# javahedi/SpinDynamics.jl

Measured on AMD Instinct MI355X. Metric: H|psi> matvecs/s, XXZ L=32 Sz=0, higher is better.
Workload: dtype c128

## Files before the change

spindynamics.jl_amd/csrc/kernels_apply.hip:

```cpp
#include <hip/hip_runtime.h>

#include <algorithm>
#include <type_traits>

#include "device_common.hpp"


using namespace sd_dev;

namespace {

template <int NC, int R, int BLOCK, bool FMA, bool PK, bool GEN = false>
__global__ __launch_bounds__(BLOCK, (GEN ? 5 : NC == 2 ? 4 : 5)) void k_apply_tiled(sd_dev_model dm, double *__restrict__ out_,
                                                       const double *__restrict__ psi_, int epi, sd_epi_args ea,
                                                       double *__restrict__ partials, int max_len) {
  using V = typename VT<NC>::type;
  constexpr uint32_t ES = sizeof(V);
  constexpr int WR = R * 64;
  extern __shared__ __attribute__((aligned(16))) unsigned char smem[];
  V *tile = reinterpret_cast<V *>(smem);
  int *lbin = reinterpret_cast<int *>(smem + (size_t)(max_len + 1) * sizeof(V));
  double *red = reinterpret_cast<double *>(lbin + 16 * SD_BIN_STRIDE);
  V *tile2 = reinterpret_cast<V *>(red + 32);

  if (ea.batch > 1) {
    const int64_t boff = (int64_t)blockIdx.y * ea.bstride * NC;
    psi_ += boff; out_ += boff;
    if (ea.prev) ea.prev = (const double *)ea.prev + boff;
    if (ea.phi) ea.phi = (const double *)ea.phi + boff;
    if (ea.accv) ea.accv = (double *)ea.accv + boff;
    partials += 2 * (size_t)blockIdx.y * (size_t)dm.n_singles;
    ea.negate = (ea.negate >> blockIdx.y) & 1;
  }
  const V *__restrict__ psi = reinterpret_cast<const V *>(psi_);
  const V *__restrict__ halo = reinterpret_cast<const V *>(ea.halo);
  const int tid = threadIdx.x;
  const int lane = tid & 63;
  const int i0 = (tid >> 6) * WR + lane;
  const int tix = blockIdx.x + dm.tile_off;
  const sd_tile_rec rec = dm.single_rec[tix];
  const uint32_t P = rec.prefix;
  const int64_t base = rec.base;
  const int p = dm.p, LS = dm.LS;
  const int len = rec.len;
  const int nU = rec.nU;
  const int nn = dm.nn_hops;
  static_assert(!GEN || PK, "general-bond plan: packed tables only");
  const bool need_sig = GEN ? (dm.need_sig_gen != 0) : (!PK || dm.need_sig);

  V own[R];
  uint32_t sig[R];
  typedef unsigned int u4 __attribute__((ext_vector_type(4)));
  u4 pt[PK ? R : 1];
  uint32_t dg[R];
  const uint32_t off0 = (uint32_t)i0 * ES;
  {
    const __amdgpu_buffer_rsrc_t rs = make_rsrc(psi + base, (uint32_t)len * ES);
#pragma unroll
    for (int r = 0; r < R; ++r) buf_load(own[r], rs, off0 + (uint32_t)(r * 64) * ES);
    if (PK && !need_sig && !dm.diag_cache) {
      const __amdgpu_buffer_rsrc_t rg = make_rsrc(dm.suf_dg + rec.suf_off, (uint32_t)len);
#pragma unroll
      for (int r = 0; r < R; ++r) dg[r] = (uint32_t)(unsigned char)__builtin_amdgcn_raw_buffer_load_b8(rg, (uint32_t)i0 + (uint32_t)(r * 64), 0, 0);
    }
    if (need_sig) {
      const __amdgpu_buffer_rsrc_t rsig = make_rsrc(dm.suf_states + rec.suf_off, (uint32_t)len * 2u);
#pragma unroll
      for (int r = 0; r < R; ++r) sig[r] = buf_load_u16(rsig, (uint32_t)i0 * 2u + (uint32_t)(r * 64) * 2u);
    } else {
#pragma unroll
      for (int r = 0; r < R; ++r) sig[r] = 0;
    }
  }

  uint64_t fmask = 0;
  int64_t my_base = -1;
  const uint32_t bitp = p >= 1 ? ((P >> (p - 1)) & 1u) : 0u;
  if (nn > 0 && p >= 1) {
    const int b = lane + 1;
    if (b <= p) my_base = dm.far_base[(size_t)tix * (size_t)p + (size_t)lane];
    fmask = __ballot(my_base >= 0);
  }
  const int st_lo = bitp ? nU : 0, st_n = bitp ? len - nU : nU;
  auto get_bond = [&](int ln) {
    FarBond fb;
    fb.base = rl64(my_base, ln); fb.J = dm.hop_J[ln];
    const bool st = ln == p - 1;
    fb.lo = st ? st_lo : 0; fb.n = st ? st_n : len;
    return fb;
  };
  constexpr bool SKIP_DEAD = NC == 1 || BLOCK == 64;
  uint32_t live = 0;
  if (SKIP_DEAD) {
#pragma unroll
    for (int r = 0; r < R; ++r)
      if ((tid & ~63) / 64 * WR + r * 64 < len) live |= 1u << r;
    live = (uint32_t)__builtin_amdgcn_readfirstlane((int)live);
  }
  auto issue = [&](const FarBond &fb, V(&v)[R]) {
    const V *__restrict__ pb = (halo && fb.base >= dm.n_local) ? halo + (fb.base - dm.n_local) : psi + fb.base;
    const __amdgpu_buffer_rsrc_t rs = make_rsrc(pb, (uint32_t)fb.n * ES);
    const uint32_t rel = off0 - (uint32_t)fb.lo * ES;
#pragma unroll
    for (int r = 0; r < R; ++r)
      if (!SKIP_DEAD || ((live >> r) & 1u)) buf_load(v[r], rs, rel + (uint32_t)(r * 64) * ES);
  };

  V va[R], vb[R];
  if (SKIP_DEAD) {
#pragma unroll
    for (int r = 0; r < R; ++r) { va[r] = V{}; vb[r] = V{}; }
  }
  FarBond fa{}, fbb{};
  uint64_t mk = fmask;
  bool have_a = false;
  auto next_lane = [&](uint64_t &m_) { const int ln = __builtin_ctzll(m_); m_ &= m_ - 1; return ln; };
  if (mk) { fa = get_bond(next_lane(mk)); issue(fa, va); have_a = true; }

  V acc[R];
  if (dm.diag_cache) {
    double dd[R];
    const __amdgpu_buffer_rsrc_t rd = make_rsrc(dm.diag_cache + base, (uint32_t)len * (uint32_t)sizeof(double));
#pragma unroll
    for (int r = 0; r < R; ++r) buf_load(dd[r], rd, (uint32_t)i0 * (uint32_t)sizeof(double) + (uint32_t)(r * 64) * (uint32_t)sizeof(double));
#pragma unroll
    for (int r = 0; r < R; ++r) acc[r] = vscale(dd[r], own[r]);
  } else if (!need_sig) {
    const int antiP = p >= 2 ? __popc((P ^ (P >> 1)) & ((1u << (p - 1)) - 1u)) : 0;
#pragma unroll
    for (int r = 0; r < R; ++r) {
      int anti = antiP + (int)(dg[r] & 15u) + (p >= 1 ? (int)(bitp ^ (dg[r] >> 4)) : 0);
      if (dm.n_zz_nn == 0) anti = 0;
      acc[r] = vscale(dm.diag_q * (double)(dm.n_zz - 2 * anti), own[r]);
    }
  } else if (dm.diag_mode == 0) {
    const DiagHead dh = diag_head(dm, P, p);
#pragma unroll
    for (int r = 0; r < R; ++r) {
      const uint64_t s = (uint64_t)P | ((uint64_t)sig[r] << p);
      acc[r] = vscale(diag_tail(dm, dh, s, p), own[r]);
    }
  } else {
#pragma unroll
    for (int r = 0; r < R; ++r) {
      const uint64_t s = (uint64_t)P | ((uint64_t)sig[r] << p);
      acc[r] = vscale(diag_of(dm, s), own[r]);
    }
  }
#pragma unroll
  for (int r = 0; r < R; ++r)
    if (i0 + r * 64 < len) tile[1 + i0 + r * 64] = own[r];
  if (tid == 0) tile[0] = V{};
  if (!PK)
    for (int k = tid; k < 16 * SD_BIN_STRIDE; k += BLOCK) {
      int n = k / SD_BIN_STRIDE, kk = k - n * SD_BIN_STRIDE;
      lbin[k] = (int)binom_g(dm, n, kk);
    }

  __syncthreads();
  while (have_a) {
    bool have_b = false;
    if (mk) { fbb = get_bond(next_lane(mk)); issue(fbb, vb); have_b = true; }
#pragma unroll
    for (int r = 0; r < R; ++r) acc[r] = accum<FMA>(acc[r], fa.J, va[r]);
    have_a = false;
    if (!have_b) break;
    if (mk) { fa = get_bond(next_lane(mk)); issue(fa, va); have_a = true; }
#pragma unroll
    for (int r = 0; r < R; ++r) acc[r] = accum<FMA>(acc[r], fbb.J, vb[r]);
  }
  if (PK && nn > 0) {
    const __amdgpu_buffer_rsrc_t rp = make_rsrc(dm.suf_part + 4 * (size_t)rec.suf_off, (uint32_t)len * 16u);
#pragma unroll
    for (int r = 0; r < R; ++r) pt[PK ? r : 0] = __builtin_amdgcn_raw_buffer_load_b128(rp, (uint32_t)i0 * 16u + (uint32_t)(r * 64) * 16u, 0, 0);
  }
  const bool wrap = !GEN && PK && !(NC == 1 && R == 8) && nn > 0 && dm.wrap_hop == nn;
  bool wrap_on = false;
  if (wrap) {
    const uint32_t Q = P ^ (1u << dm.wrap_pb);
    const int t2q = dm.nup - __popc(Q);
    if (t2q >= 0 && t2q <= LS) {
      wrap_on = true;
      const int64_t qb = dm.addr[Q];
      const int lenq = (int)dm.binom[LS * (SD_MAX_L + 1) + t2q];
      const V *__restrict__ pbq = (halo && qb >= dm.n_local) ? halo + (qb - dm.n_local) : psi + qb;
      const __amdgpu_buffer_rsrc_t rq = make_rsrc(pbq, (uint32_t)lenq * ES);
      for (int c0 = 0; c0 < lenq; c0 += BLOCK * R) {
#pragma unroll
        for (int r = 0; r < R; ++r) buf_load(va[r], rq, off0 + (uint32_t)(c0 + r * 64) * ES);
#pragma unroll
        for (int r = 0; r < R; ++r)
          if (c0 + i0 + r * 64 < lenq) tile2[1 + c0 + i0 + r * 64] = va[r];
      }
      if (tid == 0) tile2[0] = V{};
    }
  }

  struct GBond { int64_t base; uint32_t smask; int pb; int kind; };
  auto gbond = [&](int h) {
    GBond g{0, 0u, 0, -1};
    const int bi = dm.hop_i[h] - 1, bj = dm.hop_j[h] - 1;
    const bool ip = bi < p, jp = bj < p;
    if (ip && jp) {
      if (((P >> bi) ^ (P >> bj)) & 1u) { g.kind = 0; g.base = dm.addr[P ^ (1u << bi) ^ (1u << bj)]; }
    } else if (!ip && !jp) {
      g.kind = 1; g.smask = (1u << (bi - p)) | (1u << (bj - p));
    } else {
      g.pb = ip ? bi : bj;
      g.smask = 1u << ((ip ? bj : bi) - p);
      const uint32_t Q = P ^ (1u << g.pb);
      const int t2q = dm.nup - __popc(Q);
      if (t2q >= 0 && t2q <= LS) { g.kind = 2; g.base = dm.addr[Q]; }
    }
    return g;
  };
  auto gflip = [&](const GBond &g, int r) -> bool {
    if (g.kind == 0) return true;
    if (g.kind == 1) return __popc(sig[r] & g.smask) == 1;
    if (g.kind == 2) return ((P >> g.pb) & 1u) != ((sig[r] & g.smask) ? 1u : 0u);
    return false;
  };
  auto gvalue = [&](const GBond &g, int r) -> V {
    if (g.kind == 1) return tile[1 + dm.suf_rank[sig[r] ^ g.smask]];
    const int64_t idx = g.base + (g.kind == 0 ? (int64_t)(i0 + r * 64) : (int64_t)dm.suf_rank[sig[r] ^ g.smask]);
    return (halo && idx >= dm.n_local) ? halo[idx - dm.n_local] : psi[idx];
  };
  const bool have_g = !GEN && nn < dm.n_hop;
  double gJ = 0.0;
  GBond g0{0, 0u, 0, -1};
  auto request_g0 = [&]() {
    g0 = gbond(nn);
    gJ = dm.hop_J[nn];
#pragma unroll
    for (int r = 0; r < R; ++r) va[r] = (i0 + r * 64 < len && gflip(g0, r)) ? gvalue(g0, r) : V{};
  };
  if (have_g && !PK) request_g0();
  if (nn > 0) {
    if constexpr (PK) {
      const unsigned char *tb = reinterpret_cast<const unsigned char *>(tile);
      constexpr uint32_t SH = NC == 2 ? 4 : 3;
#pragma unroll
      for (int a = 1; a <= 11; ++a) if (a <= LS - 1) {
        const double J = dm.hop_J[p + a - 1];
        const int w = (a - 1) / 3, sh = 10 * ((a - 1) % 3);
        V v[R];
#pragma unroll
        for (int r = 0; r < R; ++r) {
          const u4 q = pt[PK ? r : 0];
          const uint32_t word = w == 0 ? q.x : w == 1 ? q.y : w == 2 ? q.z : q.w;
          const uint32_t ad = ((word >> sh) & 0x3FFu) << SH;
          v[r] = *reinterpret_cast<const V *>(tb + ad);
        }
#pragma unroll
        for (int r = 0; r < R; ++r) acc[r] = accum<FMA>(acc[r], J, v[r]);
      }
    } else {
      uint32_t dw[R];
#pragma unroll
      for (int r = 0; r < R; ++r) dw[r] = sig[r] ^ (sig[r] >> 1);
      for (int a = 1; a <= LS - 1; ++a) {
        const double J = dm.hop_J[p + a - 1];
        const int *brow = lbin + (LS - a - 1) * SD_BIN_STRIDE;
        int d[R];
#pragma unroll
        for (int r = 0; r < R; ++r) d[r] = brow[__popc(sig[r] >> (a + 1))];
        V v[R];
#pragma unroll
        for (int r = 0; r < R; ++r) {
          const bool up = (sig[r] >> (a - 1)) & 1u;
          const bool fl = (dw[r] >> (a - 1)) & 1u;
          const int ip = (i0 + r * 64) + (up ? d[r] : -d[r]);
          v[r] = tile[fl ? ip + 1 : 0];
        }
#pragma unroll
        for (int r = 0; r < R; ++r) acc[r] = accum<FMA>(acc[r], J, v[r]);
      }
    }
  }
  if constexpr (GEN) {
    constexpr uint32_t SH = NC == 2 ? 4 : 3;
    const unsigned char *tb = reinterpret_cast<const unsigned char *>(tile);
    const unsigned char *tb2 = reinterpret_cast<const unsigned char *>(tile2);
    uint32_t ptw[R];
    int cur_word = -1;
    auto gissue = [&](int64_t gbase, V(&v)[R]) {
      const V *__restrict__ pbp = (halo && gbase >= dm.n_local) ? halo + (gbase - dm.n_local) : psi + gbase;
      const __amdgpu_buffer_rsrc_t rs = make_rsrc(pbp, (uint32_t)len * ES);
#pragma unroll
      for (int r = 0; r < R; ++r) buf_load(v[r], rs, off0 + (uint32_t)(r * 64) * ES);
    };
    for (int hb = 0; hb < dm.n_gen; hb += 64) {
      const int nb = dm.n_gen - hb < 64 ? dm.n_gen - hb : 64;
      int64_t base_k = -1;
      sd_gbond gl{-1, 0u, 0, 0, 0.0};
      if (lane < nb) {
        gl = dm.gen[hb + lane];
        if (gl.kind == 0 && __popc(P & gl.pmask) == 1) base_k = dm.addr[P ^ gl.pmask];
      }
      uint64_t todo = __ballot(base_k >= 0);
      int in_a = -1;
      if (todo) { in_a = next_lane(todo); gissue(rl64(base_k, in_a), va); }
#pragma nounroll
      for (int k = 0; k < nb; ++k) {
        sd_gbond gb;
        gb.kind = rl(gl.kind, k); gb.pmask = (uint32_t)rl((int)gl.pmask, k); gb.slot = rl(gl.slot, k); gb.pb = rl(gl.pb, k);
        gb.J = rld(gl.J, k);
        if (gb.kind == 0) {
          if (k == in_a) {
#pragma unroll
            for (int r = 0; r < R; ++r) acc[r] = accum<false>(acc[r], gb.J, va[r]);
            in_a = -1;
            if (todo) { in_a = next_lane(todo); gissue(rl64(base_k, in_a), va); }
          }
        } else if (gb.kind == 1) {
          const int wi = gb.slot / 3, sh = 10 * (gb.slot - 3 * wi);
          if (wi != cur_word) {
            cur_word = wi;
            const int chunk = wi >> 2;
            const __amdgpu_buffer_rsrc_t rp2 = make_rsrc(dm.gen_ss_part + 4 * ((size_t)chunk * (size_t)dm.n_suf_rows + (size_t)rec.suf_off), (uint32_t)len * 16u);
            const uint32_t wo = (uint32_t)(wi & 3) * 4u;
#pragma unroll
            for (int r = 0; r < R; ++r) ptw[r] = (uint32_t)__builtin_amdgcn_raw_buffer_load_b32(rp2, (uint32_t)i0 * 16u + (uint32_t)(r * 64) * 16u + wo, 0, 0);
          }
          V v[R];
#pragma unroll
          for (int r = 0; r < R; ++r) v[r] = *reinterpret_cast<const V *>(tb + ((((ptw[r] >> sh) & 0x3FFu)) << SH));
#pragma unroll
          for (int r = 0; r < R; ++r) acc[r] = accum<false>(acc[r], gb.J, v[r]);
        } else if (gb.kind == 2) {
          const uint32_t Q = P ^ gb.pmask;
          const int t2q = dm.nup - __popc(Q);
          const bool ok = t2q >= 0 && t2q <= LS;
          __syncthreads();
          if (ok) {
            const int64_t qb = dm.addr[Q];
            const int lenq = (int)dm.binom[LS * (SD_MAX_L + 1) + t2q];
            const V *__restrict__ pbq = (halo && qb >= dm.n_local) ? halo + (qb - dm.n_local) : psi + qb;
            const __amdgpu_buffer_rsrc_t rq = make_rsrc(pbq, (uint32_t)lenq * ES);
            for (int c0 = 0; c0 < lenq; c0 += BLOCK * R) {
              V tmp[R];
#pragma unroll
              for (int r = 0; r < R; ++r) buf_load(tmp[r], rq, off0 + (uint32_t)(c0 + r * 64) * ES);
#pragma unroll
              for (int r = 0; r < R; ++r)
                if (c0 + i0 + r * 64 < lenq) tile2[1 + c0 + i0 + r * 64] = tmp[r];
            }
            if (tid == 0) tile2[0] = V{};
          }
          __syncthreads();
          if (ok) {
            const __amdgpu_buffer_rsrc_t rm = make_rsrc(dm.mix_part + ((size_t)gb.slot * (size_t)dm.n_suf_rows + (size_t)rec.suf_off), (uint32_t)len * 2u);
            const uint32_t bpb = (P >> gb.pb) & 1u;
            uint32_t w16[R];
#pragma unroll
            for (int r = 0; r < R; ++r) w16[r] = buf_load_u16(rm, (uint32_t)i0 * 2u + (uint32_t)(r * 64) * 2u);
#pragma unroll
            for (int r = 0; r < R; ++r) {
              const bool has = (w16[r] >> 15) != bpb;
              const uint32_t ad = has ? ((w16[r] & 0x3FFu) << SH) : 0u;
              acc[r] = accum<false>(acc[r], gb.J, *reinterpret_cast<const V *>(tb2 + ad));
            }
          }
        }
      }
    }
  }
  if (wrap) {
    __syncthreads();
    if (wrap_on) {
      const double Jw = dm.hop_J[nn];
      const uint32_t bpb = (P >> dm.wrap_pb) & 1u;
      const unsigned char *tb2 = reinterpret_cast<const unsigned char *>(tile2);
      constexpr uint32_t SH = NC == 2 ? 4 : 3;
#pragma unroll
      for (int r = 0; r < R; ++r) {
        const uint32_t w3 = pt[PK ? r : 0].w;
        const bool has = ((w3 >> 30) & 1u) != bpb;
        const uint32_t ad = has ? (((w3 >> 20) & 0x3FFu) << SH) : 0u;
        acc[r] = accum<false>(acc[r], Jw, *reinterpret_cast<const V *>(tb2 + ad));
      }
    }
  }
  if (have_g) {
    if (!wrap) {
      if (PK) request_g0();
#pragma unroll
      for (int r = 0; r < R; ++r)
        if (gflip(g0, r)) acc[r] = accum<false>(acc[r], gJ, va[r]);
    }
    for (int h = nn + 1; h < dm.n_hop; ++h) {
      const GBond g = gbond(h);
      if (g.kind < 0) continue;
      const double J = dm.hop_J[h];
#pragma unroll
      for (int r = 0; r < R; ++r)
        if (i0 + r * 64 < len && gflip(g, r)) acc[r] = accum<false>(acc[r], J, gvalue(g, r));
    }
  }

  EpiSums sums{0.0, 0.0};
#pragma unroll
  for (int r = 0; r < R; ++r) {
    const int i = i0 + r * 64;
    if (i < len) epilogue<NC>(epi, ea, base + i, acc[r], tile[1 + i], out_, sums);
  }
  if (epi_has_sums(epi)) {
    double a = sums.s0, b = sums.s1;
    block_reduce2(a, b, red);
    if (tid == 0) { partials[2 * (size_t)tix] = a; partials[2 * (size_t)tix + 1] = b; }
  }
}

template <int NC, bool FMA>
__global__ __launch_bounds__(256, 4) void k_apply_fulltile(sd_dev_model dm, double *__restrict__ out_,
                                                        const double *__restrict__ psi_, int epi, sd_epi_args ea,
                                                        double *__restrict__ partials) {
  using V = typename VT<NC>::type;
  constexpr uint32_t ES = sizeof(V);
  constexpr int R = 4, BLOCK = 256;
  extern __shared__ __attribute__((aligned(16))) unsigned char smem[];
  const int LF = dm.full_ls, TL = 1 << LF;
  V *tile = reinterpret_cast<V *>(smem);
  double *red = reinterpret_cast<double *>(smem + (size_t)(TL + 1) * sizeof(V));
  const V *__restrict__ psi = reinterpret_cast<const V *>(psi_);
  const V *__restrict__ halo = reinterpret_cast<const V *>(ea.halo);
  const int tid = threadIdx.x, lane = tid & 63;
  uint32_t T = blockIdx.x;
  if (gridDim.x >= 512 && (gridDim.x & 255u) == 0) {
    const uint32_t x = T & 7u, j = T >> 3, g = j >> 5, i = j & 31u;
    T = (g << 8) + (x << 5) + i;
  }
  const int64_t base = (int64_t)T << LF;
  const uint32_t Tg = T + (uint32_t)(dm.row_lo >> LF);
  const int64_t gbase = (int64_t)Tg << LF;
  const int nn = dm.nn_hops;

  V own[R];
  uint32_t ioff[R];
  {
    const __amdgpu_buffer_rsrc_t rs = make_rsrc(psi + base, (uint32_t)TL * ES);
#pragma unroll
    for (int r = 0; r < R; ++r) { ioff[r] = (uint32_t)(tid + r * BLOCK) * ES; buf_load(own[r], rs, ioff[r]); }
  }
  uint64_t fmask = 0;
  int64_t my_base = 0;
  double my_J = 0.0;
  int my_lo = 0, my_n = TL;
  if (nn > 0) {
    const int a = LF + lane;
    bool fl = false;
    if (a <= dm.L - 1) {
      if (lane == 0) {
        const int t = (int)(T & 1u);
        my_lo = (1 - t) * (TL / 2); my_n = TL / 2;
        my_base = ((int64_t)(T ^ 1u) << LF) + (TL / 2 - my_lo);
        fl = true;
      } else {
        const int b = a - LF - 1;
        fl = ((Tg >> b) ^ (Tg >> (b + 1))) & 1u;
        const uint32_t Tp = Tg ^ (3u << b);
        const int tb = dm.L - LF - dm.fs_dbits;
        const uint32_t q = Tp >> tb;
        const int64_t at_peer = (int64_t)(Tp & ((1u << tb) - 1u)) << LF;
        my_base = at_peer;
        if (q != (Tg >> tb)) {
          int64_t ho = 0, plo = 0;
#pragma unroll
          for (int q2 = 0; q2 < SD_FS_MAX_RANKS; ++q2)
            if ((uint32_t)q2 == q) { ho = dm.fs_halo_off[q2]; plo = dm.fs_peer_lo[q2]; }
          my_base = dm.n_local + ho + at_peer - plo;
        }
      }
      my_J = dm.hop_J[a - 1];
    }
    fmask = __ballot(fl);
  }
  auto get_bond = [&](int ln) {
    FarBond fb;
    fb.base = rl64(my_base, ln); fb.J = rld(my_J, ln);
    fb.lo = rl(my_lo, ln); fb.n = rl(my_n, ln);
    return fb;
  };
  auto issue = [&](const FarBond &fb, V(&v)[R]) {
    const V *__restrict__ pb = (halo && fb.base >= dm.n_local) ? halo + (fb.base - dm.n_local) : psi + fb.base;
    const __amdgpu_buffer_rsrc_t rs = make_rsrc(pb, (uint32_t)fb.n * ES);
    const uint32_t lo_b = (uint32_t)fb.lo * ES;
#pragma unroll
    for (int r = 0; r < R; ++r) buf_load(v[r], rs, ioff[r] - lo_b);
  };
  V va[R], vb[R];
  FarBond fa{}, fbb{};
  uint64_t mk = fmask;
  bool have_a = false;
  auto next_lane = [&](uint64_t &m_) { const int ln = __builtin_ctzll(m_); m_ &= m_ - 1; return ln; };
  if (mk) { fa = get_bond(next_lane(mk)); issue(fa, va); have_a = true; }

  V acc[R];
#pragma unroll
  for (int r = 0; r < R; ++r) {
    acc[r] = vscale(diag_of(dm, (uint64_t)gbase + (uint64_t)(tid + r * BLOCK)), own[r]);
    tile[tid + r * BLOCK] = own[r];
  }
  if (tid == 0) tile[TL] = V{};
  __syncthreads();

  const int n_in = nn > 0 ? LF - 1 : 0;
  for (int a = 1; a <= n_in; ++a) {
    const double J = dm.hop_J[a - 1];
    V v[R];
#pragma unroll
    for (int r = 0; r < R; ++r) {
      const int i = tid + r * BLOCK;
      const bool fl = ((i >> (a - 1)) ^ (i >> a)) & 1;
      v[r] = tile[fl ? (i ^ (3 << (a - 1))) : TL];
    }
#pragma unroll
    for (int r = 0; r < R; ++r) acc[r] = accum<FMA>(acc[r], J, v[r]);
  }
  while (have_a) {
    bool have_b = false;
    if (mk) { fbb = get_bond(next_lane(mk)); issue(fbb, vb); have_b = true; }
#pragma unroll
    for (int r = 0; r < R; ++r) acc[r] = accum<FMA>(acc[r], fa.J, va[r]);
    have_a = false;
    if (!have_b) break;
    if (mk) { fa = get_bond(next_lane(mk)); issue(fa, va); have_a = true; }
#pragma unroll
    for (int r = 0; r < R; ++r) acc[r] = accum<FMA>(acc[r], fbb.J, vb[r]);
  }
  for (int h = nn; h < dm.n_hop; ++h) {
    const int bi = dm.hop_i[h] - 1, bj = dm.hop_j[h] - 1;
    const double J = dm.hop_J[h];
#pragma unroll
    for (int r = 0; r < R; ++r) {
      const uint64_t s = (uint64_t)gbase + (uint64_t)(tid + r * BLOCK);
      if (((s >> bi) ^ (s >> bj)) & 1) acc[r] = accum<false>(acc[r], J, psi[s ^ ((uint64_t)1 << bi) ^ ((uint64_t)1 << bj)]);
    }
  }
  EpiSums sums{0.0, 0.0};
#pragma unroll
  for (int r = 0; r < R; ++r) {
    const int i = tid + r * BLOCK;
    epilogue<NC>(epi, ea, base + i, acc[r], tile[i], out_, sums);
  }
  if (epi_has_sums(epi)) {
    double a = sums.s0, b = sums.s1;
    block_reduce2(a, b, red);
    if (tid == 0) { partials[2 * (size_t)blockIdx.x] = a; partials[2 * (size_t)blockIdx.x + 1] = b; }
  }
}

template <int NC>
__global__ __launch_bounds__(256) void k_apply_generic(sd_dev_model dm, double *__restrict__ out_,
                                                       const double *__restrict__ psi_, int epi, sd_epi_args ea,
                                                       double *__restrict__ partials) {
  using V = typename VT<NC>::type;
  __shared__ double red[32];
  __shared__ int64_t lb[64 * 64];
  const V *__restrict__ psi = reinterpret_cast<const V *>(psi_);
  const bool full = dm.nup < 0;
  const int L = dm.L;
  if (!full) {
    for (int i = threadIdx.x; i < 64 * 64; i += blockDim.x) {
      const int n = i >> 6, k = i & 63;
      lb[i] = (n <= L && k <= n) ? dm.binom[n * (SD_MAX_L + 1) + k] : 0;
    }
    __syncthreads();
  }
  auto bl = [&](int n, int k) -> int64_t { return (k < 0 || k > n) ? 0 : lb[(n << 6) + k]; };
  auto unrank_l = [&](int64_t idx) {
    uint64_t s = 0;
    int r = dm.nup;
    for (int k = 1; k <= L && r > 0; ++k) {
      const int64_t c = bl(L - k, r - 1);
      if (idx < c) { s |= (uint64_t)1 << (k - 1); --r; }
      else idx -= c;
    }
    return s;
  };
  auto rank_l = [&](uint64_t s) {
    int64_t idx = 0;
    int r = dm.nup;
    for (int k = 1; k <= L && r > 0; ++k) {
      if ((s >> (k - 1)) & 1) --r;
      else idx += bl(L - k, r - 1);
    }
    return idx;
  };
  const int nn = full ? 0 : dm.nn_hops;
  EpiSums sums{0.0, 0.0};
  const int64_t stride = (int64_t)gridDim.x * blockDim.x;
  for (int64_t idx = (int64_t)blockIdx.x * blockDim.x + threadIdx.x; idx < dm.N; idx += stride) {
    const uint64_t s = full ? (uint64_t)idx : unrank_l(idx);
    const V own = psi[idx];
    V acc = vscale(diag_of(dm, s), own);
    for (int b = 1; b <= nn; ++b)
      if (((s >> (b - 1)) ^ (s >> b)) & 1) {
        const int64_t d = lb[((L - b - 1) << 6) + __popcll(s >> (b + 1))];
        const int64_t nidx = ((s >> (b - 1)) & 1) ? idx + d : idx - d;
        acc = vadd_mul(acc, dm.hop_J[b - 1], psi[nidx]);
      }
    for (int h = nn; h < dm.n_hop; ++h) {
      const int bi = dm.hop_i[h] - 1, bj = dm.hop_j[h] - 1;
      if (((s >> bi) ^ (s >> bj)) & 1) {
        const uint64_t s2 = s ^ ((uint64_t)1 << bi) ^ ((uint64_t)1 << bj);
        const int64_t nidx = full ? (int64_t)s2 : rank_l(s2);
        acc = vadd_mul(acc, dm.hop_J[h], psi[nidx]);
      }
    }
    epilogue<NC>(epi, ea, idx, acc, own, out_, sums);
  }
  if (epi_has_sums(epi)) {
    double a = sums.s0, b = sums.s1;
    block_reduce2(a, b, red);
    if (threadIdx.x == 0) { partials[2 * (size_t)blockIdx.x] = a; partials[2 * (size_t)blockIdx.x + 1] = b; }
  }
}

template <int NC, int LPT>
__global__ __launch_bounds__(256) void k_apply_short(sd_dev_model dm, double *__restrict__ out_, const double *__restrict__ psi_, int epi,
                                                     sd_epi_args ea, double *__restrict__ partials, int first, int count) {
  using V = typename VT<NC>::type;
  __shared__ int64_t lb[64 * 64];
  if (ea.batch > 1) {
    const int64_t boff = (int64_t)blockIdx.y * ea.bstride * NC;
    psi_ += boff; out_ += boff;
    if (ea.prev) ea.prev = (const double *)ea.prev + boff;
    if (ea.phi) ea.phi = (const double *)ea.phi + boff;
    if (ea.accv) ea.accv = (double *)ea.accv + boff;
    partials += 2 * (size_t)blockIdx.y * (size_t)dm.n_singles;
    ea.negate = (ea.negate >> blockIdx.y) & 1;
  }
  const V *__restrict__ psi = reinterpret_cast<const V *>(psi_);
  const int L = dm.L, p = dm.p;
  for (int i = threadIdx.x; i < 64 * 64; i += blockDim.x) {
    const int n = i >> 6, k = i & 63;
    lb[i] = (n <= L && k <= n) ? dm.binom[n * (SD_MAX_L + 1) + k] : 0;
  }
  __syncthreads();
  auto bl = [&](int n, int k) -> int64_t { return (k < 0 || k > n) ? 0 : lb[(n << 6) + k]; };
  auto rank_l = [&](uint64_t s) {
    int64_t idx = 0;
    int r = dm.nup;
    for (int k = 1; k <= L && r > 0; ++k) {
      if ((s >> (k - 1)) & 1) --r;
      else idx += bl(L - k, r - 1);
    }
    return idx;
  };
  constexpr int TPB = 256 / LPT;
  const int i = threadIdx.x % LPT;
  const int nn = dm.nn_hops;
  const int sweeps = (count + (int)gridDim.x * TPB - 1) / ((int)gridDim.x * TPB);
  for (int sw = 0; sw < sweeps; ++sw) {
    const int g = (sw * (int)gridDim.x + (int)blockIdx.x) * TPB + (int)threadIdx.x / LPT;
    const bool have_tile = g < count;
    const int tix = first + (have_tile ? g : 0);
    const sd_tile_rec rec = dm.single_rec[tix];
    EpiSums sums{0.0, 0.0};
    if (have_tile && i < rec.len) {
      const int64_t idx = rec.base + i;
      const uint64_t s = (uint64_t)rec.prefix | ((uint64_t)dm.suf_states[rec.suf_off + i] << p);
      const V own = psi[idx];
      V acc = vscale(dm.diag_cache ? dm.diag_cache[idx] : diag_of(dm, s), own);
      for (int b = 1; b <= nn; ++b)
        if (((s >> (b - 1)) ^ (s >> b)) & 1) {
          const int64_t d = lb[((L - b - 1) << 6) + __popcll(s >> (b + 1))];
          const int64_t nidx = ((s >> (b - 1)) & 1) ? idx + d : idx - d;
          acc = vadd_mul(acc, dm.hop_J[b - 1], psi[nidx]);
        }
      for (int h = nn; h < dm.n_hop; ++h) {
        const int bi = dm.hop_i[h] - 1, bj = dm.hop_j[h] - 1;
        if (((s >> bi) ^ (s >> bj)) & 1) {
          const uint64_t s2 = s ^ ((uint64_t)1 << bi) ^ ((uint64_t)1 << bj);
          acc = vadd_mul(acc, dm.hop_J[h], psi[rank_l(s2)]);
        }
      }
      epilogue<NC>(epi, ea, idx, acc, own, out_, sums);
    }
    if (epi_has_sums(epi)) {
      double a = sums.s0, b = sums.s1;
      if (LPT > 1)
        for (int off = LPT / 2; off > 0; off >>= 1) {
          a += __shfl_down(a, off, LPT);
          b += __shfl_down(b, off, LPT);
        }
      if (have_tile && i == 0) { partials[2 * (size_t)tix] = a; partials[2 * (size_t)tix + 1] = b; }
    }
  }
}

template <int NC>
__global__ __launch_bounds__(256) void k_epilogue_only(int epi, sd_epi_args ea, int64_t n, double *out_,
                                                       const double *hpsi_, const double *__restrict__ psi_,
                                                       double *__restrict__ partials) {
  using V = typename VT<NC>::type;
  __shared__ double red[32];
  const V *hpsi = reinterpret_cast<const V *>(hpsi_);
  const V *__restrict__ psi = reinterpret_cast<const V *>(psi_);
  EpiSums sums{0.0, 0.0};
  const int64_t stride = (int64_t)gridDim.x * blockDim.x;
  for (int64_t i = (int64_t)blockIdx.x * blockDim.x + threadIdx.x; i < n; i += stride) {
    const V acc = hpsi[i], own = psi[i];
    epilogue<NC>(epi, ea, i, acc, own, out_, sums);
  }
  if (epi_has_sums(epi)) {
    double a = sums.s0, b = sums.s1;
    block_reduce2(a, b, red);
    if (threadIdx.x == 0) { partials[2 * (size_t)blockIdx.x] = a; partials[2 * (size_t)blockIdx.x + 1] = b; }
  }
}

__global__ __launch_bounds__(1024) void k_reduce_pairs(const double *__restrict__ partials, int64_t n,
                                                       double *__restrict__ scalars, int64_t dstride) {
  __shared__ double red[32];
  partials += 2 * (size_t)blockIdx.x * (size_t)n;
  scalars += (size_t)blockIdx.x * (size_t)dstride;
  double a = 0.0, b = 0.0;
  for (int64_t i = threadIdx.x; i < n; i += blockDim.x) { a += partials[2 * i]; b += partials[2 * i + 1]; }
  block_reduce2(a, b, red);
  if (threadIdx.x == 0) { scalars[0] = a; scalars[1] = b; }
}

__global__ __launch_bounds__(256) void k_reduce_pairs_stage(const double *__restrict__ partials, int64_t n, int64_t chunk,
                                                            double *__restrict__ stage) {
  __shared__ double red[32];
  const int64_t lo = (int64_t)blockIdx.x * chunk, hi = lo + chunk < n ? lo + chunk : n;
  const double2 *__restrict__ p2 = reinterpret_cast<const double2 *>(partials);
  double a = 0.0, b = 0.0;
  for (int64_t i = lo + threadIdx.x; i < hi; i += blockDim.x) { const double2 v = p2[i]; a += v.x; b += v.y; }
  block_reduce2(a, b, red);
  if (threadIdx.x == 0) { stage[2 * blockIdx.x] = a; stage[2 * blockIdx.x + 1] = b; }
}

}
int sd_reduce_pairs(sd_ctx *ctx, int64_t n, double *dst) {
  if (!dst) dst = ctx->d_scalars;
  const double *src = ctx->d_partials;
  if (n > 16384) {
    double *stage = ctx->d_partials + 2 * n;
    const int64_t chunk = (n + SD_RED_STAGE_BLOCKS - 1) / SD_RED_STAGE_BLOCKS;
    hipLaunchKernelGGL(k_reduce_pairs_stage, dim3(SD_RED_STAGE_BLOCKS), dim3(256), 0, ctx->stream, src, n, chunk, stage);
    SD_HIP(ctx, hipGetLastError());
    src = stage; n = SD_RED_STAGE_BLOCKS;
  }
  hipLaunchKernelGGL(k_reduce_pairs, dim3(1), dim3(1024), 0, ctx->stream, src, n, dst, (int64_t)0);
  SD_HIP(ctx, hipGetLastError());
  return SD_OK;
}
int sd_reduce_pairs_batched(sd_ctx *ctx, int64_t n, int batch, double *dst, int64_t dstride) {
  if (!dst || n > 16384 || batch < 1) return sd_set_err(ctx, SD_EINTERNAL, "bad batched reduction");
  hipLaunchKernelGGL(k_reduce_pairs, dim3((unsigned)batch), dim3(1024), 0, ctx->stream, ctx->d_partials, n, dst, dstride);
  SD_HIP(ctx, hipGetLastError());
  return SD_OK;
}
int sd_launch_epilogue_only(sd_ctx *ctx, int dtype, int64_t n, void *out, const void *hpsi, const void *psi, int epi,
                            const sd_epi_args &ea_in) {
  const bool sums = (epi == SD_EPI_DOT || epi == SD_EPI_KPM || epi == SD_EPI_RESCALE_DOT);
  sd_epi_args ea = ea_in;
  ea.stream_hint = 0;
  if (n <= 0) {
    if (sums) SD_HIP(ctx, hipMemsetAsync(ea.sums_dst ? ea.sums_dst : ctx->d_scalars, 0, 2 * sizeof(double), ctx->stream));
    return SD_OK;
  }
  const int64_t nb = std::min<int64_t>((n + 255) / 256, 4096);
  if (sums) { int rc = sd_ensure_partials(ctx, 2 * (size_t)nb + 2 * SD_RED_STAGE_BLOCKS); if (rc) return rc; }
  if (dtype == SD_C128)
    hipLaunchKernelGGL(k_epilogue_only<2>, dim3((unsigned)nb), dim3(256), 0, ctx->stream, epi, ea, n, (double *)out,
                       (const double *)hpsi, (const double *)psi, ctx->d_partials);
  else
    hipLaunchKernelGGL(k_epilogue_only<1>, dim3((unsigned)nb), dim3(256), 0, ctx->stream, epi, ea, n, (double *)out,
                       (const double *)hpsi, (const double *)psi, ctx->d_partials);
  SD_HIP(ctx, hipGetLastError());
  if (sums) return sd_reduce_pairs(ctx, nb, ea.sums_dst);
  return SD_OK;
}
namespace {

template <int NC, int R, int BLOCK, bool FMA, bool PK, bool GEN = false>
int launch_tiled_cfg(sd_ctx *ctx, const sd_dev_model &dm, int nt, size_t shmem, double *out, const double *psi, int epi,
                     const sd_epi_args &ea, int max_len) {
  void (*kern)(sd_dev_model, double *, const double *, int, sd_epi_args, double *, int) = k_apply_tiled<NC, R, BLOCK, FMA, PK, GEN>;
  if (shmem > 48 * 1024)
    SD_HIP(ctx, hipFuncSetAttribute((const void *)kern, hipFuncAttributeMaxDynamicSharedMemorySize, (int)shmem));
  hipLaunchKernelGGL(kern, dim3(nt, ea.batch > 1 ? ea.batch : 1), dim3(BLOCK), shmem, ctx->stream, dm, out, psi, epi, ea, ctx->d_partials, max_len);
  SD_HIP(ctx, hipGetLastError());
  return SD_OK;
}

template <int NC, bool FMA>
int launch_tiled(sd_ctx *ctx, const sd_dev_model &dm, int nt, int cls, size_t shmem, double *out, const double *psi, int epi,
                 const sd_epi_args &ea, int max_len) {
  constexpr int R = 4;
  if ((64 << cls) * R < max_len) return sd_set_err(ctx, SD_EINTERNAL, "tile longer than its workgroup can hold");
  if (!dm.suf_part) {
    switch (cls) {
      case 3: return launch_tiled_cfg<NC, R, 512, FMA, false>(ctx, dm, nt, shmem, out, psi, epi, ea, max_len);
      case 4: return launch_tiled_cfg<NC, R, 1024, FMA, false>(ctx, dm, nt, shmem, out, psi, epi, ea, max_len);
    }
    return sd_set_err(ctx, SD_EINTERNAL, "bad tile length class for a plan without the packed partner table");
  }
  if (dm.n_gen > 0)
    switch (cls) {
      case 0: return launch_tiled_cfg<NC, R, 64, FMA, true, true>(ctx, dm, nt, shmem, out, psi, epi, ea, max_len);
      case 1: return launch_tiled_cfg<NC, R, 128, FMA, true, true>(ctx, dm, nt, shmem, out, psi, epi, ea, max_len);
      case 2: return launch_tiled_cfg<NC, R, 256, FMA, true, true>(ctx, dm, nt, shmem, out, psi, epi, ea, max_len);
      default: return sd_set_err(ctx, SD_EINTERNAL, "bad tile length class");
    }
  constexpr bool F8 = NC == 1;
  switch (cls) {
    case 0: return launch_tiled_cfg<NC, R, 64, FMA, true>(ctx, dm, nt, shmem, out, psi, epi, ea, max_len);
    case 1: return launch_tiled_cfg<NC, F8 ? 8 : R, F8 ? 64 : 128, FMA, true>(ctx, dm, nt, shmem, out, psi, epi, ea, max_len);
    case 2: return launch_tiled_cfg<NC, F8 ? 8 : R, F8 ? 128 : 256, FMA, true>(ctx, dm, nt, shmem, out, psi, epi, ea, max_len);
  }
  return sd_set_err(ctx, SD_EINTERNAL, "bad tile length class");
}

}

int sd_launch_apply(sd_ctx *ctx, const sd_model *m, int dtype, void *out, const void *psi, int epi,
                    const sd_epi_args &ea_in, int part) {
  if (!m->dev_ready) return sd_set_err(ctx, SD_EARG, "model has no device tables (created without a context)");
  if (dtype != SD_F64 && dtype != SD_C128) return sd_set_err(ctx, SD_EARG, "dtype must be SD_F64 or SD_C128");
  const bool sums = (epi == SD_EPI_DOT || epi == SD_EPI_KPM || epi == SD_EPI_RESCALE_DOT);
  sd_dev_model dm = m->dm;
  sd_epi_args ea = ea_in;
  ea.stream_hint = 3;
  if (dm.n_local == 0) {
    if (sums) SD_HIP(ctx, hipMemsetAsync(ea.sums_dst ? ea.sums_dst : ctx->d_scalars, 0, 2 * sizeof(double), ctx->stream));
    return SD_OK;
  }
  if (ea.no_reduce && (m->p < 0 || part != 0)) return sd_set_err(ctx, SD_EINTERNAL, "unreduced sums: whole tiled plans only");
  if (ea.batch > 1 && (m->p < 0 || m->nranks != 1 || part != 0 || dm.n_singles > 16384 || (sums && !ea.sums_dst && !ea.no_reduce)))
    return sd_set_err(ctx, SD_EINTERNAL, "batched apply: unsharded tiled plans with at most 16384 tiles only");
  if (m->p >= 0) {
    int nt = dm.n_singles;
    if (part == 1) nt = dm.n_interior;
    else if (part == 2) nt = dm.n_singles - dm.n_interior;
    if (sums) { int rc = sd_ensure_partials(ctx, 2 * (size_t)dm.n_singles * (size_t)std::max(ea.batch, 1) + 2 * SD_RED_STAGE_BLOCKS); if (rc) return rc; }
    const int max_len = m->max_tile_len;
    const size_t esz = dtype == SD_C128 ? 16 : 8;
    int rc = SD_OK;
    if (nt > 0) {
      const int s0 = part == 2 ? SD_N_LEN_CLASS : 0, s1 = part == 1 ? SD_N_LEN_CLASS : 2 * SD_N_LEN_CLASS;
      for (int sg = s0; sg < s1 && rc == SD_OK; ++sg) {
        const int cnt = m->seg_off[sg + 1] - m->seg_off[sg];
        if (cnt <= 0) continue;
        const int cls = m->seg_cls[sg];
        const int seg_max = std::min(max_len, (64 << cls) * 4);
        size_t shmem = (size_t)(seg_max + 1) * esz + 16 * SD_BIN_STRIDE * sizeof(int) + 32 * sizeof(double) + 16;
        if ((dm.wrap_hop >= 0 && dm.wrap_hop == dm.nn_hops) || dm.n_gen_mixed > 0) shmem += (size_t)(m->max_tile_len_all + 1) * esz;
        dm.tile_off = m->seg_off[sg];
        if (dtype == SD_C128)
          rc = m->hop_pow2 ? launch_tiled<2, true>(ctx, dm, cnt, cls, shmem, (double *)out, (const double *)psi, epi, ea, seg_max)
                           : launch_tiled<2, false>(ctx, dm, cnt, cls, shmem, (double *)out, (const double *)psi, epi, ea, seg_max);
        else
          rc = m->hop_pow2 ? launch_tiled<1, true>(ctx, dm, cnt, cls, shmem, (double *)out, (const double *)psi, epi, ea, seg_max)
                           : launch_tiled<1, false>(ctx, dm, cnt, cls, shmem, (double *)out, (const double *)psi, epi, ea, seg_max);
      }
      if (rc) return rc;
      if (dm.n_short > 0 && part == 0) {
        const unsigned by = ea.batch > 1 ? (unsigned)ea.batch : 1u;
        auto blocks = [](int tiles, int per_block) { return (unsigned)std::min(4096, std::max(1, (tiles + per_block - 1) / per_block)); };
        const int n16 = dm.n_short_multi, n1 = dm.n_short - dm.n_short_multi;
        if (n16 > 0) {
          if (dtype == SD_C128) hipLaunchKernelGGL((k_apply_short<2, 16>), dim3(blocks(n16, 16), by), dim3(256), 0, ctx->stream, dm, (double *)out, (const double *)psi, epi, ea, ctx->d_partials, dm.short_off, n16);
          else hipLaunchKernelGGL((k_apply_short<1, 16>), dim3(blocks(n16, 16), by), dim3(256), 0, ctx->stream, dm, (double *)out, (const double *)psi, epi, ea, ctx->d_partials, dm.short_off, n16);
        }
        if (n1 > 0) {
          if (dtype == SD_C128) hipLaunchKernelGGL((k_apply_short<2, 1>), dim3(blocks(n1, 256), by), dim3(256), 0, ctx->stream, dm, (double *)out, (const double *)psi, epi, ea, ctx->d_partials, dm.short_off + n16, n1);
          else hipLaunchKernelGGL((k_apply_short<1, 1>), dim3(blocks(n1, 256), by), dim3(256), 0, ctx->stream, dm, (double *)out, (const double *)psi, epi, ea, ctx->d_partials, dm.short_off + n16, n1);
        }
        SD_HIP(ctx, hipGetLastError());
      }
    }
    if (sums && part != 1 && !ea.no_reduce) {
      int rc2 = ea.batch > 1 ? sd_reduce_pairs_batched(ctx, (int64_t)dm.n_singles, ea.batch, ea.sums_dst, ea.sums_bstride)
                             : sd_reduce_pairs(ctx, (int64_t)dm.n_singles, ea.sums_dst);
      if (rc2) return rc2;
    }
  } else if (m->full_ls > 0) {
    if (part == 1) return SD_OK;
    const int64_t nb = dm.n_local >> m->full_ls;
    if (sums) { int rc = sd_ensure_partials(ctx, 2 * (size_t)nb + 2 * SD_RED_STAGE_BLOCKS); if (rc) return rc; }
    const size_t esz = dtype == SD_C128 ? 16 : 8;
    const size_t shmem = (((size_t)1 << m->full_ls) + 1) * esz + 32 * sizeof(double) + 16;
    void (*kf)(sd_dev_model, double *, const double *, int, sd_epi_args, double *) =
        dtype == SD_C128 ? (m->hop_pow2 ? k_apply_fulltile<2, true> : k_apply_fulltile<2, false>)
                         : (m->hop_pow2 ? k_apply_fulltile<1, true> : k_apply_fulltile<1, false>);
    hipLaunchKernelGGL(kf, dim3((unsigned)nb), dim3(256), shmem, ctx->stream, dm, (double *)out, (const double *)psi, epi, ea,
                       ctx->d_partials);
    SD_HIP(ctx, hipGetLastError());
    if (sums) {
      int rc2 = sd_reduce_pairs(ctx, (int64_t)nb, ea.sums_dst);
      if (rc2) return rc2;
    }
  } else {
    int64_t nb = (dm.N + 255) / 256;
    if (nb > 8192) nb = 8192;
    if (sums) { int rc = sd_ensure_partials(ctx, 2 * (size_t)nb + 2 * SD_RED_STAGE_BLOCKS); if (rc) return rc; }
    if (dtype == SD_C128)
      hipLaunchKernelGGL(k_apply_generic<2>, dim3((unsigned)nb), dim3(256), 0, ctx->stream, dm, (double *)out,
                         (const double *)psi, epi, ea, ctx->d_partials);
    else
      hipLaunchKernelGGL(k_apply_generic<1>, dim3((unsigned)nb), dim3(256), 0, ctx->stream, dm, (double *)out,
                         (const double *)psi, epi, ea, ctx->d_partials);
    SD_HIP(ctx, hipGetLastError());
    if (sums) {
      int rc2 = sd_reduce_pairs(ctx, (int64_t)nb, ea.sums_dst);
      if (rc2) return rc2;
    }
  }
  return SD_OK;
}
```

Baseline: 91.02.

## Use a fixed-depth software pipeline for far-bond loads in the c128 packed kernel

Adds a depth template parameter to the tiled apply kernel. For complex128 with the packed partner table, the kernel now keeps D far-bond gathers in flight through a rotating buffer array, and the diagonal-cache load is hoisted ahead of the first far loads. The launcher also pads dynamic LDS so residency is capped at a fixed number of waves per SIMD, trading occupancy for more registers per wave. Missing bonds are padded with zero-J dummy loads, which adds some redundant memory traffic, and dead-tile skipping is disabled in the pipelined path.

```diff
diff --git a/spindynamics.jl_amd/csrc/kernels_apply.hip b/spindynamics.jl_amd/csrc/kernels_apply.hip
--- a/spindynamics.jl_amd/csrc/kernels_apply.hip
+++ b/spindynamics.jl_amd/csrc/kernels_apply.hip
@@ -8,10 +8,14 @@
 
 using namespace sd_dev;
 
+constexpr int kC128StreamDepth = 2;
+constexpr int kC128WavesPerSimd = 4;
+constexpr int kLdsPerCu = 160 * 1024;
+
 namespace {
 
-template <int NC, int R, int BLOCK, bool FMA, bool PK, bool GEN = false>
-__global__ __launch_bounds__(BLOCK, (GEN ? 5 : NC == 2 ? 4 : 5)) void k_apply_tiled(sd_dev_model dm, double *__restrict__ out_,
+template <int NC, int R, int BLOCK, bool FMA, bool PK, bool GEN = false, int D = 1>
+__global__ __launch_bounds__(BLOCK, (GEN ? 5 : NC == 2 ? kC128WavesPerSimd : 5)) void k_apply_tiled(sd_dev_model dm, double *__restrict__ out_,
                                                        const double *__restrict__ psi_, int epi, sd_epi_args ea,
                                                        double *__restrict__ partials, int max_len) {
   using V = typename VT<NC>::type;
@@ -89,7 +93,7 @@
     fb.lo = st ? st_lo : 0; fb.n = st ? st_n : len;
     return fb;
   };
-  constexpr bool SKIP_DEAD = NC == 1 || BLOCK == 64;
+  constexpr bool SKIP_DEAD = (NC == 1 || BLOCK == 64) && D == 1;
   uint32_t live = 0;
   if (SKIP_DEAD) {
 #pragma unroll
@@ -106,7 +110,10 @@
       if (!SKIP_DEAD || ((live >> r) & 1u)) buf_load(v[r], rs, rel + (uint32_t)(r * 64) * ES);
   };
 
-  V va[R], vb[R];
+  static_assert(D == 1 || !GEN, "the general-bond plan keeps the one-deep far loop");
+  V vs[D >= 2 ? D : 2][R];
+  V(&va)[R] = vs[0];
+  V(&vb)[R] = vs[1];
   if (SKIP_DEAD) {
 #pragma unroll
     for (int r = 0; r < R; ++r) { va[r] = V{}; vb[r] = V{}; }
@@ -115,14 +122,29 @@
   uint64_t mk = fmask;
   bool have_a = false;
   auto next_lane = [&](uint64_t &m_) { const int ln = __builtin_ctzll(m_); m_ &= m_ - 1; return ln; };
-  if (mk) { fa = get_bond(next_lane(mk)); issue(fa, va); have_a = true; }
+  auto next_bond = [&](uint64_t &m_) {
+    FarBond fb{0, -0.0, 0, 0};
+    if (m_) fb = get_bond(next_lane(m_));
+    return fb;
+  };
+  double Js[D >= 2 ? D : 1];
+  double dd[R];
+  auto load_dd = [&]() {
+    const __amdgpu_buffer_rsrc_t rd = make_rsrc(dm.diag_cache + base, (uint32_t)len * (uint32_t)sizeof(double));
+#pragma unroll
+    for (int r = 0; r < R; ++r) buf_load(dd[r], rd, (uint32_t)i0 * (uint32_t)sizeof(double) + (uint32_t)(r * 64) * (uint32_t)sizeof(double));
+  };
+  if constexpr (D >= 2) {
+    if (dm.diag_cache) load_dd();
+#pragma unroll
+    for (int s = 0; s < D; ++s) { const FarBond fb = next_bond(mk); Js[s] = fb.J; issue(fb, vs[s]); }
+  } else {
+    if (mk) { fa = get_bond(next_lane(mk)); issue(fa, va); have_a = true; }
+  }
 
   V acc[R];
   if (dm.diag_cache) {
-    double dd[R];
-    const __amdgpu_buffer_rsrc_t rd = make_rsrc(dm.diag_cache + base, (uint32_t)len * (uint32_t)sizeof(double));
-#pragma unroll
-    for (int r = 0; r < R; ++r) buf_load(dd[r], rd, (uint32_t)i0 * (uint32_t)sizeof(double) + (uint32_t)(r * 64) * (uint32_t)sizeof(double));
+    if constexpr (D == 1) load_dd();
 #pragma unroll
     for (int r = 0; r < R; ++r) acc[r] = vscale(dd[r], own[r]);
   } else if (!need_sig) {
@@ -158,16 +180,29 @@
     }
 
   __syncthreads();
-  while (have_a) {
-    bool have_b = false;
-    if (mk) { fbb = get_bond(next_lane(mk)); issue(fbb, vb); have_b = true; }
-#pragma unroll
-    for (int r = 0; r < R; ++r) acc[r] = accum<FMA>(acc[r], fa.J, va[r]);
-    have_a = false;
-    if (!have_b) break;
-    if (mk) { fa = get_bond(next_lane(mk)); issue(fa, va); have_a = true; }
-#pragma unroll
-    for (int r = 0; r < R; ++r) acc[r] = accum<FMA>(acc[r], fbb.J, vb[r]);
+  if constexpr (D >= 2) {
+    for (int left = __popcll(fmask); left > 0; left -= D) {
+#pragma unroll
+      for (int s = 0; s < D; ++s) {
+#pragma unroll
+        for (int r = 0; r < R; ++r) acc[r] = accum<FMA>(acc[r], Js[s], vs[s][r]);
+        const FarBond fb = next_bond(mk);
+        Js[s] = fb.J;
+        issue(fb, vs[s]);
+      }
+    }
+  } else {
+    while (have_a) {
+      bool have_b = false;
+      if (mk) { fbb = get_bond(next_lane(mk)); issue(fbb, vb); have_b = true; }
+#pragma unroll
+      for (int r = 0; r < R; ++r) acc[r] = accum<FMA>(acc[r], fa.J, va[r]);
+      have_a = false;
+      if (!have_b) break;
+      if (mk) { fa = get_bond(next_lane(mk)); issue(fa, va); have_a = true; }
+#pragma unroll
+      for (int r = 0; r < R; ++r) acc[r] = accum<FMA>(acc[r], fbb.J, vb[r]);
+    }
   }
   if (PK && nn > 0) {
     const __amdgpu_buffer_rsrc_t rp = make_rsrc(dm.suf_part + 4 * (size_t)rec.suf_off, (uint32_t)len * 16u);
@@ -780,7 +815,10 @@
 template <int NC, int R, int BLOCK, bool FMA, bool PK, bool GEN = false>
 int launch_tiled_cfg(sd_ctx *ctx, const sd_dev_model &dm, int nt, size_t shmem, double *out, const double *psi, int epi,
                      const sd_epi_args &ea, int max_len) {
-  void (*kern)(sd_dev_model, double *, const double *, int, sd_epi_args, double *, int) = k_apply_tiled<NC, R, BLOCK, FMA, PK, GEN>;
+  constexpr bool PIPE = NC == 2 && PK && !GEN;
+  void (*kern)(sd_dev_model, double *, const double *, int, sd_epi_args, double *, int) = k_apply_tiled<NC, R, BLOCK, FMA, PK, GEN, PIPE ? kC128StreamDepth : 1>;
+  if (PIPE)
+    shmem = std::max(shmem, (size_t)kLdsPerCu / (size_t)(kC128WavesPerSimd * 256 / BLOCK));
   if (shmem > 48 * 1024)
     SD_HIP(ctx, hipFuncSetAttribute((const void *)kern, hipFuncAttributeMaxDynamicSharedMemorySize, (int)shmem));
   hipLaunchKernelGGL(kern, dim3(nt, ea.batch > 1 ? ea.batch : 1), dim3(BLOCK), shmem, ctx->stream, dm, out, psi, epi, ea, ctx->d_partials, max_len);
```

Result: no change. 91.19, median of 6 (+0.2%).
